# eps696/aphantasia

Hardware: AMD Instinct MI355X
Metric: optimization steps/sec @1280x720 ViT-B/32 samples=200 (higher is better)
Workload: dtype f16 (MFMA operands, fp32 accumulate; fp32 residual stream / LayerNorm / softmax statistics / synth / sampler / loss / Adam)

## Files before the change

### aphantasia_amd/_ffi.py

```python
import ctypes
import os
from ctypes import POINTER, c_char_p, c_float, c_int, c_size_t, c_void_p

import torch

HERE = os.path.dirname(os.path.abspath(__file__))
LIB_PATH = os.path.join(HERE, 'libaphantasia_hip.so')

APH_OUT_NCHW_RAW, APH_OUT_NCHW_NORM, APH_OUT_PATCH_F16, APH_GRAD_PATCH_F16, APH_OUT_PATCH_F16_HILO, APH_OUT_PATCH_F32 = 0, 1, 2, 3, 4, 5
APH_AUG_STRIDE = 16
APH_TF_FAST, APH_TF_CUSTOM, APH_TF_ELASTIC = 0, 1, 2
SIM_TYPES = {'cossim': 0, 'cos': 0, None: 0, 'mix': 1, 'ang': 2, 'dot': 3}


class SampleGeom(ctypes.Structure):
    _fields_ = [(n, c_int) for n in ('H', 'W', 'Hp', 'Wp', 'py0', 'px0', 'S', 'size', 'patch')]


_PROTOTYPES = {
    'aph_version': (c_int, []),
    'aph_last_error': (c_char_p, []),
    'aph_synth_plan_create': (c_int, [c_int, c_int, c_int, POINTER(c_void_p)]),
    'aph_synth_plan_destroy': (c_int, [c_void_p]),
    'aph_synth_fft_fwd': (c_int, [c_void_p, c_void_p, c_void_p, c_void_p, c_float, POINTER(c_float), c_int, c_void_p, c_void_p, c_void_p]),
    'aph_synth_fft_bwd': (c_int, [c_void_p, c_void_p, c_float, c_void_p, c_void_p, c_void_p, c_float, POINTER(c_float), c_int, c_void_p, c_void_p]),
    'aph_irfft2': (c_int, [c_void_p, c_void_p, c_void_p, c_void_p]),
    'aph_rfft2': (c_int, [c_void_p, c_void_p, c_void_p, c_void_p]),
    'aph_synth_spatial_fwd': (c_int, [c_void_p, c_void_p, c_float, c_float, POINTER(c_float), c_int, c_void_p, c_void_p]),
    'aph_synth_spatial_bwd': (c_int, [c_void_p, c_void_p, c_float, c_void_p, c_void_p, c_float, c_float, POINTER(c_float), c_int, c_void_p, c_void_p]),
    'aph_synth_stats': (c_int, [c_void_p, c_void_p, c_void_p]),
    'aph_synth_set_stats': (c_int, [c_void_p, c_void_p, c_void_p]),
    'aph_synth_plan_describe': (c_int, [c_void_p, POINTER(c_int)]),
    'aph_idwt_coarse_levels': (c_int, [POINTER(c_int), POINTER(c_int), c_int, c_int]),
    'aph_rgb_priors_ws_bytes': (c_size_t, []),
    'aph_rgb_sharp': (c_int, [c_void_p, c_int, c_int, c_float, c_void_p, c_void_p, c_void_p, c_void_p]),
    'aph_rgb_priors': (c_int, [c_void_p, c_int, c_int, c_float, c_float, c_float, c_void_p, c_void_p, c_void_p, c_void_p]),
    'aph_cppn_param_count': (c_size_t, [c_int, c_int, c_int]),
    'aph_cppn_ws_bytes': (c_size_t, [c_int, c_int, c_int, c_int, c_int]),
    'aph_cppn_fwd': (c_int, [c_void_p, c_int, c_int, c_int, c_void_p, c_void_p, c_int, c_int, c_void_p, c_void_p, c_void_p]),
    'aph_cppn_bwd': (c_int, [c_void_p, c_int, c_int, c_int, c_void_p, c_void_p, c_int, c_int, c_void_p, c_float, c_void_p, c_void_p, c_void_p, c_void_p]),
    'aph_idwt_level_fwd': (c_int, [c_void_p, c_int, c_int, c_void_p, c_int, c_int, c_int, c_void_p, c_void_p, c_int, c_float, c_void_p, c_void_p]),
    'aph_idwt_fwd': (c_int, [c_void_p, c_void_p, c_void_p, c_void_p, c_void_p, c_int, c_int, c_void_p, c_void_p, c_int, c_void_p, c_void_p]),
    'aph_idwt_bwd': (c_int, [c_void_p, c_void_p, c_void_p, c_void_p, c_int, c_int, c_void_p, c_void_p, c_int, c_void_p, c_void_p, c_void_p, c_void_p]),
    'aph_idwt_level_bwd': (c_int, [c_void_p, c_int, c_int, c_int, c_void_p, c_void_p, c_int, c_float, c_void_p, c_int, c_int, c_void_p, c_void_p]),
    'aph_sample_ws_bytes': (c_size_t, [POINTER(SampleGeom), c_int]),
    'aph_sample_fwd': (c_int, [POINTER(SampleGeom), c_void_p, c_void_p, c_void_p, c_void_p, c_void_p, c_int, c_void_p]),
    'aph_sample_bwd': (c_int, [POINTER(SampleGeom), c_void_p, c_float, c_void_p, c_void_p, c_void_p, c_void_p, c_int, c_void_p]),
    'aph_sample_ws_bytes_tf': (c_size_t, [POINTER(SampleGeom), c_int]),
    'aph_sample_fwd_tf': (c_int, [POINTER(SampleGeom), c_int, c_void_p, c_void_p, c_void_p, c_void_p, c_void_p, c_void_p, c_int, c_void_p]),
    'aph_sample_bwd_tf': (c_int, [POINTER(SampleGeom), c_int, c_void_p, c_float, c_void_p, c_void_p, c_void_p, c_void_p, c_void_p, c_int, c_void_p]),
    'aph_triangle_blur': (c_int, [c_void_p, c_int, c_int, c_int, c_int, c_float, c_float, c_void_p, c_void_p]),
    'aph_resize_bicubic': (c_int, [c_void_p, c_int, c_int, c_int, c_void_p, c_int, c_int, c_void_p]),
    'aph_flip_w': (c_int, [c_void_p, c_void_p, c_int, c_int, c_int, c_void_p, c_void_p]),
    'aph_grid_warp': (c_int, [c_void_p, c_void_p, c_int, c_int, c_int, c_float, c_float, c_float, c_float, c_float, c_void_p, c_void_p, c_void_p]),
    'aph_attn_test': (c_int, [c_void_p, c_void_p, c_void_p, c_void_p, c_void_p, c_void_p, c_int, c_int, c_int, c_int, c_void_p]),
    'aph_attn_f32_test': (c_int, [c_void_p, c_void_p, c_void_p, c_void_p, c_void_p, c_void_p, c_int, c_int, c_int, c_int, c_void_p]),
    'aph_attn_causal_f32_test': (c_int, [c_void_p, c_void_p, c_void_p, c_int, c_int, c_int, c_void_p]),
    'aph_text_create': (c_int, [c_int, c_int, c_int, c_int, c_int, c_int, c_int, POINTER(c_void_p)]),
    'aph_text_destroy': (c_int, [c_void_p]),
    'aph_text_workspace_bytes': (c_size_t, [c_void_p]),
    'aph_text_set_weight': (c_int, [c_void_p, c_char_p, c_void_p, c_size_t]),
    'aph_text_forward': (c_int, [c_void_p, c_void_p, c_int, c_void_p, c_void_p]),
    'aph_lpips_create': (c_int, [POINTER(c_int), c_int, c_int, POINTER(c_void_p)]),
    'aph_lpips_destroy': (c_int, [c_void_p]),
    'aph_lpips_workspace_bytes': (c_size_t, [c_void_p]),
    'aph_lpips_set_weight': (c_int, [c_void_p, c_char_p, c_void_p, c_size_t]),
    'aph_lpips_set_target': (c_int, [c_void_p, c_void_p, c_int, c_int, c_void_p]),
    'aph_lpips_value_grad': (c_int, [c_void_p, c_void_p, c_void_p, c_void_p, c_void_p, c_void_p]),
    'aph_lpips_value_grad_half': (c_int, [c_void_p, c_void_p, c_void_p, c_void_p, c_void_p, c_void_p]),
    'aph_lpips_pack_test': (c_int, [c_void_p, c_int, c_int, c_int, c_void_p, c_size_t]),
    'aph_lpips_conv_test': (c_int, [c_void_p, c_int, c_int, c_int, c_void_p, c_int, c_void_p, c_int, c_void_p, c_void_p, c_void_p, c_int, c_int, c_void_p]),
    'aph_lpips_pool_test': (c_int, [c_void_p, c_int, c_int, c_int, c_void_p, c_void_p, c_void_p, c_void_p]),
    'aph_lpips_head_test': (c_int, [c_void_p, c_void_p, c_void_p, c_int, c_int, c_float, c_void_p, c_void_p, c_void_p, c_void_p, c_void_p]),
    'aph_lpips_resize_test': (c_int, [c_void_p, c_int, c_int, c_void_p, c_int, c_void_p]),
    'aph_frame_affine': (c_int, [c_void_p, c_int, c_int, c_int, POINTER(c_float), c_void_p, c_void_p]),
    'aph_patchify_f16': (c_int, [c_void_p, c_int, c_int, c_int, c_void_p, c_void_p]),
    'aph_patchify_f16_hilo': (c_int, [c_void_p, c_int, c_int, c_int, c_void_p, c_void_p]),
    'aph_patchify_f32': (c_int, [c_void_p, c_int, c_int, c_int, c_void_p, c_void_p]),
    'aph_unpatchify_f32': (c_int, [c_void_p, c_int, c_int, c_int, c_float, c_void_p, c_void_p]),
    'aph_patch_row_elems': (c_int, [c_int]),
    'aph_patchify_f16_win': (c_int, [c_void_p, c_int, c_int, c_int, c_int, c_void_p, c_void_p]),
    'aph_unpatchify_f32_win': (c_int, [c_void_p, c_int, c_int, c_int, c_int, c_float, c_void_p, c_void_p]),
    'aph_vit_create': (c_int, [c_int, c_int, c_int, c_int, c_int, c_int, c_int, POINTER(c_void_p)]),
    'aph_vit_destroy': (c_int, [c_void_p]),
    'aph_vit_workspace_bytes': (c_size_t, [c_void_p]),
    'aph_vit_set_weight': (c_int, [c_void_p, c_char_p, c_void_p, c_size_t]),
    'aph_vit_forward': (c_int, [c_void_p, c_void_p, c_int, c_void_p, c_void_p]),
    'aph_vit_forward_hilo': (c_int, [c_void_p, c_void_p, c_int, c_void_p, c_void_p]),
    'aph_vit_enable_hilo': (c_int, [c_void_p]),
    'aph_vit_enable_f32': (c_int, [c_void_p]),
    'aph_vit_forward_f32': (c_int, [c_void_p, c_void_p, c_int, c_void_p, c_void_p]),
    'aph_vit_backward_f32': (c_int, [c_void_p, c_void_p, c_int, c_void_p, c_float, c_void_p]),
    'aph_vit_backward': (c_int, [c_void_p, c_void_p, c_int, c_void_p, c_float, c_void_p]),
    'aph_vit_backward_h': (c_int, [c_void_p, c_void_p, c_int, c_void_p, c_float, c_void_p]),
    'aph_vit_profile': (c_int, [c_void_p, c_int]),
    'aph_vit_profile_read': (c_int, [c_void_p, c_void_p, c_void_p, c_void_p]),
    'aph_gemm_set_mfma32': (c_int, [c_int]),
    'aph_vit_set_fuse_ln': (c_int, [c_int]),
    'aph_crop_adjoint_set_gather': (c_int, [c_int]),
    'aph_crop_adjoint_set_shape': (c_int, [c_int, c_int, c_int, c_int, c_int]),
    'aph_vit_set_grad_stream_f16': (c_int, [c_int]),
    'aph_gemm_set_ws_min_tiles': (c_int, [c_int]),
    'aph_gemm_set_ws_pgroup': (c_int, [c_int]),
    'aph_gemm_set_rs': (c_int, [c_int]),
    'aph_mfma_rate': (c_int, [c_int, c_int, c_void_p, c_void_p, c_void_p]),
    'aph_gemm_rs_probe': (c_int, [c_void_p, c_void_p, c_int, c_int, c_int, c_void_p, c_int, c_void_p, c_void_p]),
    'aph_gemm_ws_probe': (c_int, [c_void_p, c_void_p, c_int, c_int, c_int, c_void_p, c_void_p, c_void_p, c_int, c_void_p, c_void_p]),
    'aph_gemm_f32_test': (c_int, [c_void_p, c_int, c_int, c_void_p, c_int, c_int, c_int, c_int, c_void_p, c_int, c_void_p, c_void_p, c_int, c_void_p, c_size_t, c_void_p]),
    'aph_gemm_f16': (c_int, [c_void_p, c_void_p, c_int, c_int, c_int, c_void_p, c_void_p]),
    'aph_gemm_f16_ld': (c_int, [c_void_p, c_int, c_void_p, c_int, c_int, c_int, c_int, c_void_p, c_int, c_void_p]),
    'aph_gemm_f16_epi_test': (c_int, [c_void_p, c_int, c_void_p, c_int, c_int, c_int, c_int, c_void_p, c_int, c_void_p, c_void_p, c_void_p, c_float, c_int,
                                      c_int, c_int, c_int, c_void_p, c_size_t, c_int, c_void_p]),
    'aph_ln_test': (c_int, [c_int, c_int, c_int, c_int, c_int, c_int, c_int, c_void_p, c_void_p, c_void_p, c_void_p, c_void_p, c_void_p, c_void_p,
                            c_void_p, c_void_p, c_void_p, c_void_p, c_void_p, c_void_p, c_void_p]),
    'aph_sim_loss': (c_int, [c_void_p, c_int, c_int, c_void_p, c_void_p, POINTER(c_float), c_int, c_int, c_int, c_int, c_int, c_float, c_float, c_void_p, c_void_p, c_void_p, c_void_p]),
    'aph_axpy_f32': (c_int, [c_void_p, c_void_p, c_float, c_size_t, c_void_p]),
    'aph_rgb_to_u8': (c_int, [c_void_p, c_int, c_int, c_float, c_void_p, c_void_p]),
    'aph_linear_head': (c_int, [c_void_p, c_int, c_int, c_void_p, c_float, c_float, c_float, c_float, c_void_p, c_void_p, c_void_p]),
    'aph_comm_unique_id': (c_int, [c_void_p]),
    'aph_comm_init': (c_int, [c_int, c_int, c_void_p, POINTER(c_void_p)]),
    'aph_allreduce_f32': (c_int, [c_void_p, c_void_p, c_size_t, c_void_p]),
    'aph_comm_ranks': (c_int, [c_void_p, POINTER(c_int)]),
    'aph_comm_destroy': (c_int, [c_void_p]),
    'aph_adam_step': (c_int, [c_void_p, c_void_p, c_void_p, c_void_p, c_void_p, c_void_p, c_int, c_size_t, c_void_p]),
    'aph_adam_step_guarded': (c_int, [c_void_p, c_void_p, c_void_p, c_void_p, c_void_p, c_void_p, c_int, c_size_t, c_void_p, c_void_p]),
}

EXPORTS = tuple(_PROTOTYPES)

class Library:

    def __init__(self, path):
        if not os.path.isfile(path):
            raise RuntimeError(
                "aphantasia_amd: HIP library not found at %s -- build it with "
                "`python -c 'import __graft_entry__ as g; g.build()'` (hipcc, gfx950). "
                "There is no CPU fallback." % path)
        self.path = path
        self.cdll = ctypes.CDLL(path)
        for name, (res, args) in _PROTOTYPES.items():
            fn = getattr(self.cdll, name)
            fn.restype = res
            fn.argtypes = args

    def last_error(self):
        return (self.cdll.aph_last_error() or b'').decode(errors='replace')

    def call(self, name, *args):
        rc = getattr(self.cdll, name)(*args)
        if rc < 0:
            raise RuntimeError('%s failed (%d): %s' % (name, rc, self.last_error()))
        return rc


_lib = None


def lib():
    global _lib
    if _lib is None:
        import torch
        if torch.cuda.is_available():
            torch.cuda.init()
            torch.empty(1, device='cuda')
        _lib = Library(LIB_PATH)
    return _lib


def ptr(t):
    return c_void_p(t.data_ptr()) if t is not None else c_void_p(0)


def floats(seq):
    if seq is None:
        return None
    arr = (c_float * len(seq))(*[float(v) for v in seq])
    return arr
```

### aphantasia_amd/csrc/synth.hip

```cpp
#include "synth_fft.h"
#include "synth_rgb.h"
#include "synth_terms.h"
#include "synth_cppn.h"

#include <memory>

using namespace aph;

static const int kElemBlocks = 1024;

struct aph_synth_plan {
  int C, H, W, Wc, TC, col_threads = 1024;
  Fft1D ph, pw;
  int col_blocks, nrow_blocks;
  size_t col_lds, row_lds;
  float norm;
  float2 *twH = nullptr, *twW = nullptr;
  float2* tmp = nullptr;
  float* dn = nullptr;
  double* partials = nullptr;
  float* stats = nullptr;
  float* bstats = nullptr;
  size_t HW() const { return (size_t)H * W; }
  double n() const { return (double)C * H * W; }
  ~aph_synth_plan() {
    for (void* q : {(void*)twH, (void*)twW, (void*)tmp, (void*)dn, (void*)partials, (void*)stats, (void*)bstats}) (void)hipFree(q);
  }
};

static bool factorize(int n, Fft1D* p) {
  p->n = n; p->npass = 0;
  int m = n;
  auto push = [&](int r) { if (p->npass >= 14) return false; p->radix[p->npass++] = r; return true; };
  while (m % 4 == 0) { if (!push(4)) return false; m /= 4; }
  while (m % 2 == 0) { if (!push(2)) return false; m /= 2; }
  for (int r = 3; (long long)r * r <= m || r <= 31; r += 2)
    while (m % r == 0) { if (!push(r)) return false; m /= r; }
  if (m > 1 && !push(m)) return false;
  return true;
}

template <typename T>
static bool dev_alloc(T** p, size_t n) { return hipMalloc((void**)p, sizeof(T) * n) == hipSuccess; }

static float2* make_twiddles(int n) {
  std::vector<float2> h(n);
  for (int t = 0; t < n; ++t) {
    const double ang = 2.0 * M_PI * (double)t / (double)n;
    h[t] = make_float2((float)cos(ang), (float)sin(ang));
  }
  float2* d = nullptr;
  if (!dev_alloc(&d, n)) return nullptr;
  if (hipMemcpy(d, h.data(), sizeof(float2) * n, hipMemcpyHostToDevice) != hipSuccess) { (void)hipFree(d); return nullptr; }
  return d;
}

static void launch_col_synth(const aph_synth_plan* p, const float* spectrum, const float* scale, const float* shift, hipStream_t st) {
  APH_LAUNCH(fft_col_synth_kernel, dim3(p->col_blocks), dim3(p->col_threads), p->col_lds, st, (const float2*)spectrum, scale, shift, p->tmp,
             p->ph, (const float2*)p->twH, p->C, p->H, p->Wc, p->TC);
}
static void launch_row_synth(const aph_synth_plan* p, float* image, hipStream_t st) {
  APH_LAUNCH(fft_row_synth_kernel, dim3(p->nrow_blocks), dim3(256), p->row_lds, st, (const float2*)p->tmp, image, p->partials, p->pw,
             (const float2*)p->twW, p->H, p->W, p->Wc, p->norm);
}
static void launch_row_adjoint(const aph_synth_plan* p, const float* dn, const float* raw, int plain, hipStream_t st) {
  APH_LAUNCH(fft_row_adjoint_kernel, dim3(p->nrow_blocks), dim3(256), p->row_lds, st, dn, raw, plain ? (const float*)nullptr : (const float*)p->bstats,
             p->tmp, p->pw, (const float2*)p->twW, p->H, p->W, p->Wc, p->norm, plain);
}
static void launch_col_adjoint(const aph_synth_plan* p, const float* scale, float* spectrum, hipStream_t st) {
  APH_LAUNCH(fft_col_adjoint_kernel, dim3(p->col_blocks), dim3(p->col_threads), p->col_lds, st, (const float2*)p->tmp, scale, (float2*)spectrum,
             p->ph, (const float2*)p->twH, p->C, p->H, p->Wc, p->TC);
}
static void launch_stats_finalize(const aph_synth_plan* p, int nparts, hipStream_t st) {
  APH_LAUNCH(stats_finalize_kernel, dim3(1), dim3(256), 0, st, (const double*)p->partials, nparts, p->n(), p->stats);
}

static ColorMat to_cm(const float* cc) { ColorMat m; for (int i = 0; i < 9; ++i) m.m[i] = cc ? cc[i] : (i % 4 == 0 ? 1.f : 0.f); return m; }

static void launch_rgb_fwd(const aph_synth_plan* p, const float* raw, float contrast, float fixed_div, const float* colcorr_t9, int decorrelate,
                           float* rgb, hipStream_t st) {
  APH_LAUNCH(rgb_fwd_kernel, dim3(kElemBlocks), dim3(256), 0, st, raw, (const float*)p->stats, contrast, fixed_div, to_cm(colcorr_t9),
             decorrelate, rgb, p->HW());
}
static void launch_rgb_bwd(const aph_synth_plan* p, const float* d_rgb, float gscale, const float* rgb, const float* raw, float contrast,
                           float fixed_div, const float* colcorr_t9, int decorrelate, hipStream_t st) {
  APH_LAUNCH(rgb_bwd_kernel, dim3(kElemBlocks), dim3(256), 0, st, d_rgb, rgb, raw, to_cm(colcorr_t9), decorrelate, gscale, p->dn,
             p->partials, p->HW());
  APH_LAUNCH(bstats_finalize_kernel, dim3(1), dim3(256), 0, st, (const double*)p->partials, kElemBlocks, p->n(), (const float*)p->stats,
             contrast, fixed_div, p->bstats);
}

struct CppnArgs {
  const float *params, *xs, *ys;
  int W;
  size_t HW;
  CppnLayout g;
  hipStream_t st;
};
template <int ACT>
static void launch_cppn_fwd(const CppnNet& net, const CppnArgs& a, float* stash, float* rgb) {
  const size_t lds = sizeof(float) * net.fwd_lds();
  APH_ALLOW_SMEM(cppn_fwd_kernel<ACT>, lds);
  APH_LAUNCH(cppn_fwd_kernel<ACT>, dim3(a.g.ntiles < kCppnFwdBlocks ? a.g.ntiles : kCppnFwdBlocks), dim3(64 * kCppnWaves), lds, a.st, a.params, net,
             a.xs, a.ys, a.W, a.HW, stash, rgb, a.g.ntiles);
}
template <int ACT>
static void launch_cppn_bwd(const CppnNet& net, const CppnArgs& a, const float* d_rgb, float gscale, const float* rgb, const float* stash,
                            float* partials) {
  const size_t lds = sizeof(float) * net.bwd_lds();
  APH_ALLOW_SMEM(cppn_bwd_kernel<ACT>, lds);
  APH_LAUNCH(cppn_bwd_kernel<ACT>, dim3(a.g.bwd_blocks), dim3(64 * kCppnWaves), lds, a.st, a.params, net, a.xs, a.ys, a.W, a.HW, d_rgb, gscale,
             rgb, stash, partials, net.count(), a.g.ntiles);
}

extern "C" {

int aph_synth_plan_create(int C, int H, int W, aph_synth_plan** out) {
  APH_TRY
  if (!out || C < 1 || H < 2 || W < 2) return aph_fail(APH_ERR_ARG, "aph_synth_plan_create: bad shape C=%d H=%d W=%d", C, H, W);
  std::unique_ptr<aph_synth_plan> p(new aph_synth_plan());
  p->C = C; p->H = H; p->W = W; p->Wc = W / 2 + 1;
  if (!factorize(H, &p->ph) || !factorize(W, &p->pw))
    return aph_fail(APH_ERR_UNSUPPORTED, "FFT size %dx%d has more than 14 prime factors", W, H);
  if (W > 8192 || H > 8192) return aph_fail(APH_ERR_UNSUPPORTED, "FFT dimension > 8192 not supported (%dx%d)", W, H);
  int tc = (64 * 1024) / (H * 8);
  p->TC = tc < 1 ? 1 : (tc > 8 ? 8 : tc);
  p->col_blocks = (C * p->Wc + p->TC - 1) / p->TC;
  p->nrow_blocks = C * ((H + 1) / 2);
  p->col_lds = sizeof(float2) * 2 * p->TC * H;
  p->row_lds = sizeof(float2) * 2 * W;
  p->norm = (float)(1.0 / sqrt((double)H * (double)W));
  const int npart = p->nrow_blocks > kElemBlocks ? p->nrow_blocks : kElemBlocks;
  const bool ok = (p->twH = make_twiddles(H)) && (p->twW = make_twiddles(W)) && dev_alloc(&p->tmp, (size_t)C * H * p->Wc) &&
                  dev_alloc(&p->dn, (size_t)C * H * W) && dev_alloc(&p->partials, 2 * (size_t)npart) && dev_alloc(&p->stats, 2) &&
                  dev_alloc(&p->bstats, 4);
  if (!ok) return aph_fail(APH_ERR_HIP, "synth plan allocation failed");
  APH_ALLOW_SMEM(fft_col_synth_kernel, p->col_lds);
  APH_ALLOW_SMEM(fft_col_adjoint_kernel, p->col_lds);
  APH_ALLOW_SMEM(fft_row_synth_kernel, p->row_lds);
  APH_ALLOW_SMEM(fft_row_adjoint_kernel, p->row_lds);
  *out = p.release();
  return APH_OK;
  APH_CATCH
}

int aph_synth_plan_destroy(aph_synth_plan* p) {
  delete p;
  return APH_OK;
}

int aph_synth_plan_describe(const aph_synth_plan* p, int* out31) {
  APH_TRY
  if (!p || !out31) return aph_fail(APH_ERR_ARG, "aph_synth_plan_describe: null argument");
  out31[0] = p->TC;
  const Fft1D* plans[2] = {&p->ph, &p->pw};
  for (int a = 0; a < 2; ++a) {
    int* o = out31 + 1 + 15 * a;
    o[0] = plans[a]->npass;
    for (int i = 0; i < 14; ++i) o[1 + i] = i < plans[a]->npass ? plans[a]->radix[i] : 0;
  }
  return APH_OK;
  APH_CATCH
}

int aph_synth_fft_fwd(aph_synth_plan* p, const float* params, const float* scale, const float* shift, float contrast,
                      const float* colcorr_t9, int decorrelate, float* raw, float* rgb, void* stream_) {
  APH_TRY
  if (!p || !params || !scale || !raw || !rgb) return aph_fail(APH_ERR_ARG, "aph_synth_fft_fwd: null argument");
  hipStream_t st = (hipStream_t)stream_;
  launch_col_synth(p, params, scale, shift, st);
  launch_row_synth(p, raw, st);
  launch_stats_finalize(p, p->nrow_blocks, st);
  launch_rgb_fwd(p, raw, contrast, 0.f, colcorr_t9, decorrelate, rgb, st);
  return aph_check_launch("aph_synth_fft_fwd");
  APH_CATCH
}

int aph_synth_fft_bwd(aph_synth_plan* p, const float* d_rgb, float gscale, const float* rgb, const float* raw,
                      const float* scale, float contrast, const float* colcorr_t9, int decorrelate, float* grad_params,
                      void* stream_) {
  APH_TRY
  if (!p || !d_rgb || !rgb || !raw || !scale || !grad_params) return aph_fail(APH_ERR_ARG, "aph_synth_fft_bwd: null argument");
  hipStream_t st = (hipStream_t)stream_;
  launch_rgb_bwd(p, d_rgb, gscale, rgb, raw, contrast, 0.f, colcorr_t9, decorrelate, st);
  launch_row_adjoint(p, p->dn, raw, 0, st);
  launch_col_adjoint(p, scale, grad_params, st);
  return aph_check_launch("aph_synth_fft_bwd");
  APH_CATCH
}

int aph_irfft2(aph_synth_plan* p, const float* spectrum, float* image, void* stream_) {
  APH_TRY
  if (!p || !spectrum || !image) return aph_fail(APH_ERR_ARG, "aph_irfft2: null argument");
  hipStream_t st = (hipStream_t)stream_;
  launch_col_synth(p, spectrum, nullptr, nullptr, st);
  launch_row_synth(p, image, st);
  return aph_check_launch("aph_irfft2");
  APH_CATCH
}

int aph_rfft2(aph_synth_plan* p, const float* image, float* spectrum, void* stream_) {
  APH_TRY
  if (!p || !image || !spectrum) return aph_fail(APH_ERR_ARG, "aph_rfft2: null argument");
  hipStream_t st = (hipStream_t)stream_;
  launch_row_adjoint(p, image, image, 1, st);
  launch_col_adjoint(p, nullptr, spectrum, st);
  return aph_check_launch("aph_rfft2");
  APH_CATCH
}

int aph_synth_spatial_fwd(aph_synth_plan* p, const float* raw, float contrast, float fixed_div, const float* colcorr_t9,
                          int decorrelate, float* rgb, void* stream_) {
  APH_TRY
  if (!p || !raw || !rgb) return aph_fail(APH_ERR_ARG, "aph_synth_spatial_fwd: null argument");
  hipStream_t st = (hipStream_t)stream_;
  APH_LAUNCH(stats_partial_kernel, dim3(kElemBlocks, 1), dim3(256), 0, st, raw, (size_t)p->C * p->HW(), p->partials);
  launch_stats_finalize(p, kElemBlocks, st);
  launch_rgb_fwd(p, raw, contrast, fixed_div, colcorr_t9, decorrelate, rgb, st);
  return aph_check_launch("aph_synth_spatial_fwd");
  APH_CATCH
}

int aph_synth_spatial_bwd(aph_synth_plan* p, const float* d_rgb, float gscale, const float* rgb, const float* raw,
                          float contrast, float fixed_div, const float* colcorr_t9, int decorrelate, float* d_raw,
                          void* stream_) {
  APH_TRY
  if (!p || !d_rgb || !rgb || !raw || !d_raw) return aph_fail(APH_ERR_ARG, "aph_synth_spatial_bwd: null argument");
  hipStream_t st = (hipStream_t)stream_;
  launch_rgb_bwd(p, d_rgb, gscale, rgb, raw, contrast, fixed_div, colcorr_t9, decorrelate, st);
  APH_LAUNCH(norm_bwd_kernel, dim3(kElemBlocks), dim3(256), 0, st, (const float*)p->dn, raw, (const float*)p->bstats, d_raw, (size_t)p->C * p->HW());
  return aph_check_launch("aph_synth_spatial_bwd");
  APH_CATCH
}

int aph_synth_stats(aph_synth_plan* p, float* out2, void* stream_) {
  APH_TRY
  if (!p || !out2) return aph_fail(APH_ERR_ARG, "aph_synth_stats: null argument");
  if (hipMemcpyAsync(out2, p->stats, 2 * sizeof(float), hipMemcpyDeviceToDevice, (hipStream_t)stream_) != hipSuccess)
    return aph_fail(APH_ERR_HIP, "aph_synth_stats: copy failed");
  return APH_OK;
  APH_CATCH
}

int aph_synth_set_stats(aph_synth_plan* p, const float* in2, void* stream_) {
  APH_TRY
// ... 78 lines not shown
```

### aphantasia_amd/csrc/synth_fft.h

```cpp
#pragma once
#include "synth_rgb.h"

namespace aph {

struct Fft1D {
  int n, npass;
  int radix[14];
};

__device__ __forceinline__ float2 cmul(float2 a, float2 b) {
  return make_float2(a.x * b.x - a.y * b.y, a.x * b.y + a.y * b.x);
}
__device__ __forceinline__ float2 cadd(float2 a, float2 b) { return make_float2(a.x + b.x, a.y + b.y); }
__device__ __forceinline__ float2 csub(float2 a, float2 b) { return make_float2(a.x - b.x, a.y - b.y); }
template <int SIGN>
__device__ __forceinline__ float2 cmuli(float2 a) {
  return SIGN > 0 ? make_float2(-a.y, a.x) : make_float2(a.y, -a.x);
}
template <int SIGN>
__device__ __forceinline__ float2 twiddle(const float2* __restrict__ tw, int t) {
  float2 w = tw[t];
  if (SIGN < 0) w.y = -w.y;
  return w;
}

struct Butterfly {
  const float2* x;
  float2* y;
  int k;
  __device__ __forceinline__ Butterfly(const float2* src, float2* dst, int N, int R, int Ns, int q, int j)
      : x(src + q * N + j), y(dst + q * N + (j / Ns) * Ns * R + j % Ns), k(j % Ns) {}
};

template <int SIGN, int RT>
__device__ __forceinline__ void fft_pass(const float2* src, float2* dst, int N, int R_, int Ns, int nseq,
                                         const float2* __restrict__ tw) {
  const int R = RT ? RT : R_;
  const int nb = N / R, tscale = N / (Ns * R);
  for (int idx = threadIdx.x; idx < nb * nseq; idx += blockDim.x) {
    const int q = idx / nb;
    const Butterfly bf(src, dst, N, R, Ns, q, idx - q * nb);
    float2 v[RT ? RT : 32];
    for (int r = 0; r < R; ++r) {
      v[r] = bf.x[r * nb];
      if (r > 0) v[r] = cmul(v[r], twiddle<SIGN>(tw, bf.k * r * tscale));
    }
    if (RT == 2) {
      bf.y[0] = cadd(v[0], v[1]);
      bf.y[Ns] = csub(v[0], v[1]);
    } else if (RT == 3) {
      const float2 s = cadd(v[1], v[2]);
      const float2 t = make_float2(v[0].x - 0.5f * s.x, v[0].y - 0.5f * s.y);
      float2 u = csub(v[1], v[2]);
      u = cmuli<SIGN>(make_float2(u.x * 0.86602540378443865f, u.y * 0.86602540378443865f));
      bf.y[0] = cadd(v[0], s);
      bf.y[Ns] = cadd(t, u);
      bf.y[2 * Ns] = csub(t, u);
    } else if (RT == 4) {
      const float2 a0 = cadd(v[0], v[2]), a1 = csub(v[0], v[2]);
      const float2 a2 = cadd(v[1], v[3]), a3 = cmuli<SIGN>(csub(v[1], v[3]));
      bf.y[0] = cadd(a0, a2);
      bf.y[Ns] = cadd(a1, a3);
      bf.y[2 * Ns] = csub(a0, a2);
      bf.y[3 * Ns] = csub(a1, a3);
    } else {
      for (int qq = 0; qq < R; ++qq) {
        float2 acc = v[0];
        for (int r = 1; r < R; ++r) acc = cadd(acc, cmul(v[r], twiddle<SIGN>(tw, ((qq * r) % R) * nb)));
        bf.y[qq * Ns] = acc;
      }
    }
  }
}

template <int SIGN>
__device__ void fft_pass_large(const float2* src, float2* dst, int N, int R, int Ns, int nseq, const float2* __restrict__ tw) {
  const int nb = N / R, tscale = N / (Ns * R);
  for (int idx = threadIdx.x; idx < N * nseq; idx += blockDim.x) {
    const int q = idx / N, o = idx - q * N;
    const int qq = o / nb;
    const Butterfly bf(src, dst, N, R, Ns, q, o - qq * nb);
    const float2* x = bf.x;
    double ar = x[0].x, ai = x[0].y;
    const int step = (int)(((long long)bf.k * tscale + (long long)qq * nb) % N);
    int t = 0;
    for (int r = 1; r < R; ++r) {
      t += step; if (t >= N) t -= N;
      const float2 pr = cmul(x[r * nb], twiddle<SIGN>(tw, t));
      ar += pr.x; ai += pr.y;
    }
    bf.y[qq * Ns] = make_float2((float)ar, (float)ai);
  }
}

template <int SIGN>
__device__ float2* fft_lds(float2* a, float2* b, const Fft1D& plan, int nseq, const float2* __restrict__ tw) {
  int Ns = 1;
  const int N = plan.n;
  for (int p = 0; p < plan.npass; ++p) {
    const int R = plan.radix[p];
    switch (R) {
      case 2: fft_pass<SIGN, 2>(a, b, N, R, Ns, nseq, tw); break;
      case 3: fft_pass<SIGN, 3>(a, b, N, R, Ns, nseq, tw); break;
      case 4: fft_pass<SIGN, 4>(a, b, N, R, Ns, nseq, tw); break;
      case 5: fft_pass<SIGN, 5>(a, b, N, R, Ns, nseq, tw); break;
      default:
        if (R <= 31) fft_pass<SIGN, 0>(a, b, N, R, Ns, nseq, tw);
        else fft_pass_large<SIGN>(a, b, N, R, Ns, nseq, tw);
        break;
    }
    __syncthreads();
    float2* t = a; a = b; b = t;
    Ns *= R;
  }
  return a;
}

constexpr int kLoadBatch = 8;

struct ColElem {
  bool in_tile, valid;
  int lds;
  int plane;
  size_t global;
  __device__ __forceinline__ ColElem(int idx, int C, int H, int Wc, int TC) {
    const int t = idx % TC, y = idx / TC, g = blockIdx.x * TC + t;
    in_tile = idx < TC * H;
    valid = in_tile && g < C * Wc;
    const int c = valid ? g / Wc : 0, kx = valid ? g - c * Wc : 0;
    lds = t * H + y;
    plane = (valid ? y : 0) * Wc + kx;
    global = (size_t)c * H * Wc + plane;
  }
};

struct RowPair {
  size_t row0, row1, row1_or_0;
  bool has1;
  __device__ __forceinline__ explicit RowPair(int H) {
    const int pairs = (H + 1) / 2, c = blockIdx.x / pairs, y0 = 2 * (blockIdx.x - c * pairs);
    has1 = y0 + 1 < H;
    row0 = (size_t)c * H + y0;
    row1 = row0 + 1;
    row1_or_0 = has1 ? row1 : row0;
  }
};

__global__ void fft_col_synth_kernel(const float2* __restrict__ params, const float* __restrict__ scale,
                                     const float* __restrict__ shift, float2* __restrict__ tmp, Fft1D plan,
                                     const float2* __restrict__ tw, int C, int H, int Wc, int TC) {
  APH_DYN_SMEM(smem);
  float2* a = reinterpret_cast<float2*>(smem);
  float2* b = a + TC * H;
  for (int base = 0; base < TC * H; base += kLoadBatch * blockDim.x) {
    float2 v[kLoadBatch];
    float sc[kLoadBatch], sf[kLoadBatch];
#pragma unroll
    for (int u = 0; u < kLoadBatch; ++u) {
      const ColElem e(base + u * blockDim.x + threadIdx.x, C, H, Wc, TC);
      v[u] = params[e.global];
      sc[u] = scale ? scale[e.plane] : 1.0f;
      sf[u] = shift ? shift[e.plane] : 0.f;
    }
#pragma unroll
    for (int u = 0; u < kLoadBatch; ++u) {
      const ColElem e(base + u * blockDim.x + threadIdx.x, C, H, Wc, TC);
      if (e.in_tile) {
        float2 w = make_float2(0.f, 0.f);
        if (e.valid) {
          const float s = sc[u];
          w = v[u];
          w.x *= s; w.y *= s;
          if (shift) { const float sh = s * sf[u]; w.x += sh; w.y += sh; }
        }
        a[e.lds] = w;
      }
    }
  }
  __syncthreads();
  const float2* r = fft_lds<+1>(a, b, plan, TC, tw);
  for (int idx = threadIdx.x; idx < TC * H; idx += blockDim.x) {
    const ColElem e(idx, C, H, Wc, TC);
    if (e.valid) tmp[e.global] = r[e.lds];
  }
}

__global__ void fft_col_adjoint_kernel(const float2* __restrict__ tmp, const float* __restrict__ scale,
                                       float2* __restrict__ grad, Fft1D plan, const float2* __restrict__ tw,
                                       int C, int H, int Wc, int TC) {
  APH_DYN_SMEM(smem);
  float2* a = reinterpret_cast<float2*>(smem);
  float2* b = a + TC * H;
  for (int base = 0; base < TC * H; base += kLoadBatch * blockDim.x) {
    float2 v[kLoadBatch];
#pragma unroll
    for (int u = 0; u < kLoadBatch; ++u) v[u] = tmp[ColElem(base + u * blockDim.x + threadIdx.x, C, H, Wc, TC).global];
#pragma unroll
    for (int u = 0; u < kLoadBatch; ++u) {
      const ColElem e(base + u * blockDim.x + threadIdx.x, C, H, Wc, TC);
      if (e.in_tile) a[e.lds] = e.valid ? v[u] : make_float2(0.f, 0.f);
    }
  }
  __syncthreads();
  const float2* r = fft_lds<-1>(a, b, plan, TC, tw);
  for (int idx = threadIdx.x; idx < TC * H; idx += blockDim.x) {
    const ColElem e(idx, C, H, Wc, TC);
    if (e.valid) {
      const float s = scale ? scale[e.plane] : 1.0f;
      const float2 v = r[e.lds];
      grad[e.global] = make_float2(v.x * s, v.y * s);
    }
  }
}

__global__ void fft_row_synth_kernel(const float2* __restrict__ tmp, float* __restrict__ raw,
                                     double* __restrict__ partials, Fft1D plan, const float2* __restrict__ tw,
                                     int H, int W, int Wc, float norm) {
  APH_DYN_SMEM(smem);
  float2* a = reinterpret_cast<float2*>(smem);
  float2* b = a + W;
  __shared__ double red[16];
  const RowPair rp(H);
  const float2* ra = tmp + rp.row0 * Wc;
  const float2* rb = tmp + rp.row1_or_0 * Wc;
  for (int base = 0; base < Wc; base += kLoadBatch * blockDim.x) {
    float2 Av[kLoadBatch], Bw[kLoadBatch];
#pragma unroll
    for (int u = 0; u < kLoadBatch; ++u) {
      const int k = base + u * blockDim.x + threadIdx.x, kc = k < Wc ? k : 0;
      Av[u] = ra[kc];
      Bw[u] = rb[kc];
    }
#pragma unroll
    for (int u = 0; u < kLoadBatch; ++u) {
      const int k = base + u * blockDim.x + threadIdx.x;
      if (k < Wc) {
        const float2 A = Av[u];
        const float2 Bv = rp.has1 ? Bw[u] : make_float2(0.f, 0.f);
        const bool edge = (k == 0) || (2 * k == W);
        if (edge) {
          a[k] = make_float2(A.x, Bv.x);
        } else {
          a[k] = make_float2(A.x - Bv.y, A.y + Bv.x);
          a[W - k] = make_float2(A.x + Bv.y, Bv.x - A.y);
        }
      }
    }
  }
  __syncthreads();
  const float2* r = fft_lds<+1>(a, b, plan, 1, tw);
  SumSq s;
  float* o0 = raw + rp.row0 * W;
  float* o1 = raw + rp.row1 * W;
  for (int x = threadIdx.x; x < W; x += blockDim.x) {
    const float2 z = r[x];
    const float v0 = z.x * norm, v1 = z.y * norm;
    o0[x] = v0;
    s.add(v0);
    if (rp.has1) { o1[x] = v1; s.add(v1); }
  }
  s.store_block_total(red, partials + 2 * blockIdx.x);
}

__global__ void fft_row_adjoint_kernel(const float* __restrict__ dn, const float* __restrict__ raw,
                                       const float* __restrict__ bstats, float2* __restrict__ tmp, Fft1D plan,
                                       const float2* __restrict__ tw, int H, int W, int Wc, float norm, int plain) {
  APH_DYN_SMEM(smem);
  float2* a = reinterpret_cast<float2*>(smem);
  float2* b = a + W;
  const RowPair rp(H);
  const float A = plain ? 1.0f : bstats[0], Bc = plain ? 0.0f : bstats[1], mu = plain ? 0.0f : bstats[2];
  const size_t o0 = rp.row0 * W, o1c = rp.row1_or_0 * W;
  for (int base = 0; base < W; base += kLoadBatch * blockDim.x) {
    float d0[kLoadBatch], r0[kLoadBatch], d1[kLoadBatch], r1[kLoadBatch];
#pragma unroll
    for (int u = 0; u < kLoadBatch; ++u) {
      const int x = base + u * blockDim.x + threadIdx.x, xc = x < W ? x : 0;
      d0[u] = dn[o0 + xc]; r0[u] = raw[o0 + xc];
      d1[u] = dn[o1c + xc]; r1[u] = raw[o1c + xc];
    }
#pragma unroll
    for (int u = 0; u < kLoadBatch; ++u) {
      const int x = base + u * blockDim.x + threadIdx.x;
      if (x < W) {
        const float g0 = A * d0[u] + Bc * (r0[u] - mu);
        const float g1 = rp.has1 ? A * d1[u] + Bc * (r1[u] - mu) : 0.f;
        a[x] = make_float2(g0, g1);
      }
    }
  }
  __syncthreads();
  const float2* r = fft_lds<-1>(a, b, plan, 1, tw);
  float2* t0 = tmp + rp.row0 * Wc;
  float2* t1 = tmp + rp.row1 * Wc;
  for (int k = threadIdx.x; k < Wc; k += blockDim.x) {
    const float2 z = r[k];
    const float2 zc = r[k == 0 ? 0 : W - k];
    const float f = ((!plain && k >= 1 && k <= W - Wc) ? 1.0f : 0.5f) * norm;
    t0[k] = make_float2((z.x + zc.x) * f, (z.y - zc.y) * f);
    if (rp.has1) t1[k] = make_float2((z.y + zc.y) * f, (zc.x - z.x) * f);
  }
}

}
```

Measured before the change: 178.3.

## Add small-radix FFT path with fast division and LDS-staged twiddles

Adds a templated SMALL variant of the synth column and row FFT kernels for sizes whose radices are all at most 5 (e.g. 720 and 1280). It precomputes magic-multiplier divisors to replace integer division in pass indexing and tile mapping. It stages the twiddle tables into LDS with async global-to-LDS loads, and restructures the column tile so each thread owns one column and strides over rows. This targets index arithmetic and global twiddle reads in the image-parameterisation FFTs, at the cost of extra LDS per block (possibly lower occupancy) and fast-division range checks.

```diff
diff --git a/aphantasia_amd/_ffi.py b/aphantasia_amd/_ffi.py
--- a/aphantasia_amd/_ffi.py
+++ b/aphantasia_amd/_ffi.py
@@ -98,6 +98,7 @@
     'aph_gemm_set_mfma32': (c_int, [c_int]),
     'aph_vit_set_fuse_ln': (c_int, [c_int]),
     'aph_crop_adjoint_set_gather': (c_int, [c_int]),
+    'aph_synth_set_generic_passes': (c_int, [c_int]),
     'aph_crop_adjoint_set_shape': (c_int, [c_int, c_int, c_int, c_int, c_int]),
     'aph_vit_set_grad_stream_f16': (c_int, [c_int]),
     'aph_gemm_set_ws_min_tiles': (c_int, [c_int]),
diff --git a/aphantasia_amd/csrc/synth.hip b/aphantasia_amd/csrc/synth.hip
--- a/aphantasia_amd/csrc/synth.hip
+++ b/aphantasia_amd/csrc/synth.hip
@@ -3,6 +3,8 @@
 #include "synth_terms.h"
 #include "synth_cppn.h"
 
+#include <algorithm>
+#include <initializer_list>
 #include <memory>
 
 using namespace aph;
@@ -14,6 +16,8 @@
   Fft1D ph, pw;
   int col_blocks, nrow_blocks;
   size_t col_lds, row_lds;
+  bool col_small = false, row_small = false;
+  FastDiv by_tc, by_wc, by_pairs;
   float norm;
   float2 *twH = nullptr, *twW = nullptr;
   float2* tmp = nullptr;
@@ -37,16 +41,41 @@
   for (int r = 3; (long long)r * r <= m || r <= 31; r += 2)
     while (m % r == 0) { if (!push(r)) return false; m /= r; }
   if (m > 1 && !push(m)) return false;
+  p->small = 1;
+  for (int i = 0, ns = 1; i < p->npass; ns *= p->radix[i++]) {
+    p->by_nb[i] = fast_div(n / p->radix[i]);
+    p->by_ns[i] = fast_div(ns);
+    if (p->radix[i] > 5) p->small = 0;
+  }
+  return true;
+}
+
+static bool fast_div_holds(FastDiv d, unsigned long long n_end) { return d.d == 1 || n_end * d.d <= (1ull << 32); }
+
+static const size_t kLdsBytes = 160 * 1024;
+
+static int& generic_passes() {
+  static int v = 0;
+  return v;
+}
+
+static bool small_plan(const Fft1D& f, size_t lds, unsigned long long idx_end, std::initializer_list<FastDiv> dividers) {
+  if (!f.small || lds + sizeof(float2) * tw_padded(f.n) > kLdsBytes) return false;
+  for (int i = 0; i < f.npass; ++i)
+    if (!fast_div_holds(f.by_nb[i], idx_end) || !fast_div_holds(f.by_ns[i], idx_end)) return false;
+  for (FastDiv d : dividers)
+    if (!fast_div_holds(d, idx_end)) return false;
   return true;
 }
 
 template <typename T>
 static bool dev_alloc(T** p, size_t n) { return hipMalloc((void**)p, sizeof(T) * n) == hipSuccess; }
 
-static float2* make_twiddles(int n) {
-  std::vector<float2> h(n);
-  for (int t = 0; t < n; ++t) {
-    const double ang = 2.0 * M_PI * (double)t / (double)n;
+static float2* make_twiddles(int n_) {
+  const int n = tw_padded(n_);
+  std::vector<float2> h(n, make_float2(0.f, 0.f));
+  for (int t = 0; t < n_; ++t) {
+    const double ang = 2.0 * M_PI * (double)t / (double)n_;
     h[t] = make_float2((float)cos(ang), (float)sin(ang));
   }
   float2* d = nullptr;
@@ -55,21 +84,29 @@
   return d;
 }
 
+#define APH_LAUNCH_FFT(kern, small, ...)                            \
+  do {                                                              \
+    if ((small) && !generic_passes()) { APH_LAUNCH(kern<true>, __VA_ARGS__); } \
+    else { APH_LAUNCH(kern<false>, __VA_ARGS__); }                  \
+  } while (0)
+static ColTile col_tile(const aph_synth_plan* p) { return ColTile{p->C, p->H, p->Wc, p->TC, p->col_threads / p->TC, p->by_tc, p->by_wc}; }
+
 static void launch_col_synth(const aph_synth_plan* p, const float* spectrum, const float* scale, const float* shift, hipStream_t st) {
-  APH_LAUNCH(fft_col_synth_kernel, dim3(p->col_blocks), dim3(p->col_threads), p->col_lds, st, (const float2*)spectrum, scale, shift, p->tmp,
-             p->ph, (const float2*)p->twH, p->C, p->H, p->Wc, p->TC);
+  APH_LAUNCH_FFT(fft_col_synth_kernel, p->col_small, dim3(p->col_blocks), dim3(p->col_threads), p->col_lds, st, (const float2*)spectrum, scale,
+                 shift, p->tmp, p->ph, (const float2*)p->twH, col_tile(p));
 }
 static void launch_row_synth(const aph_synth_plan* p, float* image, hipStream_t st) {
-  APH_LAUNCH(fft_row_synth_kernel, dim3(p->nrow_blocks), dim3(256), p->row_lds, st, (const float2*)p->tmp, image, p->partials, p->pw,
-             (const float2*)p->twW, p->H, p->W, p->Wc, p->norm);
+  APH_LAUNCH_FFT(fft_row_synth_kernel, p->row_small, dim3(p->nrow_blocks), dim3(256), p->row_lds, st, (const float2*)p->tmp, image, p->partials,
+                 p->pw, (const float2*)p->twW, p->H, p->W, p->Wc, p->norm, p->by_pairs);
 }
 static void launch_row_adjoint(const aph_synth_plan* p, const float* dn, const float* raw, int plain, hipStream_t st) {
-  APH_LAUNCH(fft_row_adjoint_kernel, dim3(p->nrow_blocks), dim3(256), p->row_lds, st, dn, raw, plain ? (const float*)nullptr : (const float*)p->bstats,
-             p->tmp, p->pw, (const float2*)p->twW, p->H, p->W, p->Wc, p->norm, plain);
+  APH_LAUNCH_FFT(fft_row_adjoint_kernel, p->row_small, dim3(p->nrow_blocks), dim3(256), p->row_lds, st, dn, raw,
+                 plain ? (const float*)nullptr : (const float*)p->bstats, p->tmp, p->pw, (const float2*)p->twW, p->H, p->W, p->Wc, p->norm, plain,
+                 p->by_pairs);
 }
 static void launch_col_adjoint(const aph_synth_plan* p, const float* scale, float* spectrum, hipStream_t st) {
-  APH_LAUNCH(fft_col_adjoint_kernel, dim3(p->col_blocks), dim3(p->col_threads), p->col_lds, st, (const float2*)p->tmp, scale, (float2*)spectrum,
-             p->ph, (const float2*)p->twH, p->C, p->H, p->Wc, p->TC);
+  APH_LAUNCH_FFT(fft_col_adjoint_kernel, p->col_small, dim3(p->col_blocks), dim3(p->col_threads), p->col_lds, st, (const float2*)p->tmp, scale,
+                 (float2*)spectrum, p->ph, (const float2*)p->twH, col_tile(p));
 }
 static void launch_stats_finalize(const aph_synth_plan* p, int nparts, hipStream_t st) {
   APH_LAUNCH(stats_finalize_kernel, dim3(1), dim3(256), 0, st, (const double*)p->partials, nparts, p->n(), p->stats);
@@ -129,16 +166,23 @@
   p->nrow_blocks = C * ((H + 1) / 2);
   p->col_lds = sizeof(float2) * 2 * p->TC * H;
   p->row_lds = sizeof(float2) * 2 * W;
+  p->by_tc = fast_div(p->TC); p->by_wc = fast_div(p->Wc); p->by_pairs = fast_div((H + 1) / 2);
+  const unsigned long long col_end = std::max<unsigned long long>({(unsigned long long)p->col_threads, (unsigned long long)p->TC * H,
+                                                                   (unsigned long long)C * p->Wc + p->TC});
+  p->col_small = small_plan(p->ph, p->col_lds, col_end, {p->by_tc, p->by_wc});
+  p->row_small = small_plan(p->pw, p->row_lds, std::max<unsigned long long>(W, p->nrow_blocks), {p->by_pairs});
+  if (p->col_small) p->col_lds += sizeof(float2) * tw_padded(H);
+  if (p->row_small) p->row_lds += sizeof(float2) * tw_padded(W);
   p->norm = (float)(1.0 / sqrt((double)H * (double)W));
   const int npart = p->nrow_blocks > kElemBlocks ? p->nrow_blocks : kElemBlocks;
   const bool ok = (p->twH = make_twiddles(H)) && (p->twW = make_twiddles(W)) && dev_alloc(&p->tmp, (size_t)C * H * p->Wc) &&
                   dev_alloc(&p->dn, (size_t)C * H * W) && dev_alloc(&p->partials, 2 * (size_t)npart) && dev_alloc(&p->stats, 2) &&
                   dev_alloc(&p->bstats, 4);
   if (!ok) return aph_fail(APH_ERR_HIP, "synth plan allocation failed");
-  APH_ALLOW_SMEM(fft_col_synth_kernel, p->col_lds);
-  APH_ALLOW_SMEM(fft_col_adjoint_kernel, p->col_lds);
-  APH_ALLOW_SMEM(fft_row_synth_kernel, p->row_lds);
-  APH_ALLOW_SMEM(fft_row_adjoint_kernel, p->row_lds);
+  APH_ALLOW_SMEM(fft_col_synth_kernel<true>, p->col_lds);   APH_ALLOW_SMEM(fft_col_synth_kernel<false>, p->col_lds);
+  APH_ALLOW_SMEM(fft_col_adjoint_kernel<true>, p->col_lds); APH_ALLOW_SMEM(fft_col_adjoint_kernel<false>, p->col_lds);
+  APH_ALLOW_SMEM(fft_row_synth_kernel<true>, p->row_lds);   APH_ALLOW_SMEM(fft_row_synth_kernel<false>, p->row_lds);
+  APH_ALLOW_SMEM(fft_row_adjoint_kernel<true>, p->row_lds); APH_ALLOW_SMEM(fft_row_adjoint_kernel<false>, p->row_lds);
   *out = p.release();
   return APH_OK;
   APH_CATCH
@@ -161,6 +205,12 @@
   }
   return APH_OK;
   APH_CATCH
+}
+
+int aph_synth_set_generic_passes(int on) {
+  const int prev = generic_passes();
+  generic_passes() = on ? 1 : 0;
+  return prev;
 }
 
 int aph_synth_fft_fwd(aph_synth_plan* p, const float* params, const float* scale, const float* shift, float contrast,
diff --git a/aphantasia_amd/csrc/synth_fft.h b/aphantasia_amd/csrc/synth_fft.h
--- a/aphantasia_amd/csrc/synth_fft.h
+++ b/aphantasia_amd/csrc/synth_fft.h
@@ -2,10 +2,18 @@
 #include "synth_rgb.h"
 
 namespace aph {
+
+struct FastDiv {
+  uint32_t d, m;
+  __host__ __device__ __forceinline__ int quot(int n) const { return d == 1 ? n : (int)(((uint64_t)(uint32_t)n * m) >> 32); }
+};
+inline FastDiv fast_div(int d) { return FastDiv{(uint32_t)d, d > 1 ? (uint32_t)((1ull << 32) / (uint32_t)d) + 1u : 0u}; }
 
 struct Fft1D {
   int n, npass;
   int radix[14];
+  FastDiv by_nb[14], by_ns[14];
+  int small;
 };
 
 __device__ __forceinline__ float2 cmul(float2 a, float2 b) {
@@ -93,21 +101,81 @@
   }
 }
 
-template <int SIGN>
-__device__ float2* fft_lds(float2* a, float2* b, const Fft1D& plan, int nseq, const float2* __restrict__ tw) {
+template <int SIGN, int R>
+__device__ __forceinline__ void fft_pass_small(const float2* src, float2* dst, int N, int Ns, int nseq, const float2* tw, FastDiv by_nb,
+                                               FastDiv by_ns) {
+  const int nb = (int)by_nb.d, tscale = by_ns.quot(nb);
+  float2 root[R];
+  if (R == 5) {
+#pragma unroll
+    for (int m = 0; m < R; ++m) root[m] = twiddle<SIGN>(tw, m * nb);
+  }
+  for (int idx = threadIdx.x; idx < nb * nseq; idx += blockDim.x) {
+    const int q = nseq == 1 ? 0 : by_nb.quot(idx), j = idx - q * nb;
+    const int blk = by_ns.quot(j), k = j - blk * Ns;
+    const float2* x = src + q * N + j;
+    float2* y = dst + q * N + blk * Ns * R + k;
+    float2 v[R];
+#pragma unroll
+    for (int r = 0; r < R; ++r) {
+      v[r] = x[r * nb];
+      if (r > 0) v[r] = cmul(v[r], twiddle<SIGN>(tw, k * r * tscale));
+    }
+    if (R == 2) {
+      y[0] = cadd(v[0], v[1]);
+      y[Ns] = csub(v[0], v[1]);
+    } else if (R == 3) {
+      const float2 s = cadd(v[1], v[2]);
+      const float2 t = make_float2(v[0].x - 0.5f * s.x, v[0].y - 0.5f * s.y);
+      float2 u = csub(v[1], v[2]);
+      u = cmuli<SIGN>(make_float2(u.x * 0.86602540378443865f, u.y * 0.86602540378443865f));
+      y[0] = cadd(v[0], s);
+      y[Ns] = cadd(t, u);
+      y[2 * Ns] = csub(t, u);
+    } else if (R == 4) {
+      const float2 a0 = cadd(v[0], v[2]), a1 = csub(v[0], v[2]);
+      const float2 a2 = cadd(v[1], v[3]), a3 = cmuli<SIGN>(csub(v[1], v[3]));
+      y[0] = cadd(a0, a2);
+      y[Ns] = cadd(a1, a3);
+      y[2 * Ns] = csub(a0, a2);
+      y[3 * Ns] = csub(a1, a3);
+    } else {
+#pragma unroll
+      for (int qq = 0; qq < R; ++qq) {
+        float2 acc = v[0];
+#pragma unroll
+        for (int r = 1; r < R; ++r) acc = cadd(acc, cmul(v[r], root[(qq * r) % R]));
+        y[qq * Ns] = acc;
+      }
+    }
+  }
+}
+
+template <int SIGN, bool SMALL>
+__device__ float2* fft_lds(float2* a, float2* b, const Fft1D& plan, int nseq, const float2* tw) {
   int Ns = 1;
   const int N = plan.n;
   for (int p = 0; p < plan.npass; ++p) {
     const int R = plan.radix[p];
-    switch (R) {
-      case 2: fft_pass<SIGN, 2>(a, b, N, R, Ns, nseq, tw); break;
-      case 3: fft_pass<SIGN, 3>(a, b, N, R, Ns, nseq, tw); break;
-      case 4: fft_pass<SIGN, 4>(a, b, N, R, Ns, nseq, tw); break;
-      case 5: fft_pass<SIGN, 5>(a, b, N, R, Ns, nseq, tw); break;
-      default:
-        if (R <= 31) fft_pass<SIGN, 0>(a, b, N, R, Ns, nseq, tw);
-        else fft_pass_large<SIGN>(a, b, N, R, Ns, nseq, tw);
-        break;
+    if (SMALL) {
+      const FastDiv by_nb = plan.by_nb[p], by_ns = plan.by_ns[p];
+      switch (R) {
+        case 2: fft_pass_small<SIGN, 2>(a, b, N, Ns, nseq, tw, by_nb, by_ns); break;
+        case 3: fft_pass_small<SIGN, 3>(a, b, N, Ns, nseq, tw, by_nb, by_ns); break;
+        case 4: fft_pass_small<SIGN, 4>(a, b, N, Ns, nseq, tw, by_nb, by_ns); break;
+        default: fft_pass_small<SIGN, 5>(a, b, N, Ns, nseq, tw, by_nb, by_ns); break;
+      }
+    } else {
+      switch (R) {
+        case 2: fft_pass<SIGN, 2>(a, b, N, R, Ns, nseq, tw); break;
+        case 3: fft_pass<SIGN, 3>(a, b, N, R, Ns, nseq, tw); break;
+        case 4: fft_pass<SIGN, 4>(a, b, N, R, Ns, nseq, tw); break;
+        case 5: fft_pass<SIGN, 5>(a, b, N, R, Ns, nseq, tw); break;
+        default:
+          if (R <= 31) fft_pass<SIGN, 0>(a, b, N, R, Ns, nseq, tw);
+          else fft_pass_large<SIGN>(a, b, N, R, Ns, nseq, tw);
+          break;
+      }
     }
     __syncthreads();
     float2* t = a; a = b; b = t;
@@ -118,27 +186,58 @@
 
 constexpr int kLoadBatch = 8;
 
-struct ColElem {
-  bool in_tile, valid;
-  int lds;
-  int plane;
-  size_t global;
-  __device__ __forceinline__ ColElem(int idx, int C, int H, int Wc, int TC) {
-    const int t = idx % TC, y = idx / TC, g = blockIdx.x * TC + t;
-    in_tile = idx < TC * H;
-    valid = in_tile && g < C * Wc;
-    const int c = valid ? g / Wc : 0, kx = valid ? g - c * Wc : 0;
-    lds = t * H + y;
-    plane = (valid ? y : 0) * Wc + kx;
-    global = (size_t)c * H * Wc + plane;
-  }
-};
-
+template <bool SMALL>
+__device__ __forceinline__ int quot(int n, FastDiv d) { return SMALL ? d.quot(n) : n / (int)d.d; }
+
+constexpr int kTwChunk = 128;
+__host__ __device__ __forceinline__ int tw_padded(int n) { return (n + kTwChunk - 1) / kTwChunk * kTwChunk; }
+template <bool SMALL>
+__device__ __forceinline__ const float2* stage_twiddles(const float2* __restrict__ tw, float2* lds, int n) {
+  if (!SMALL) return tw;
+  const int wave = wave_uniform(threadIdx.x >> 6), nw = blockDim.x >> 6, lane = threadIdx.x & 63;
+  for (int c = wave * kTwChunk; c < n; c += nw * kTwChunk) glds16(tw + c + 2 * lane, lds + c);
+  return lds;
+}
+__device__ __forceinline__ void wait_twiddles() {
+#ifndef APH_EMU
+  asm volatile("s_waitcnt vmcnt(0)" ::: "memory");
+#endif
+}
+
+struct ColTile {
+  int C, H, Wc, TC, rows;
+  FastDiv by_tc, by_wc;
+};
+
+template <bool SMALL>
+struct ColThread {
+  bool active, valid;
+  int y0, rows, H, Wc;
+  int lds0;
+  int kx;
+  size_t global0;
+  __device__ __forceinline__ explicit ColThread(const ColTile& g) : rows(g.rows), H(g.H), Wc(g.Wc) {
+    y0 = quot<SMALL>(threadIdx.x, g.by_tc);
+    const int t = threadIdx.x - y0 * g.TC, col = blockIdx.x * g.TC + t;
+    active = y0 < rows;
+    valid = active && col < g.C * g.Wc;
+    const int c = valid ? quot<SMALL>(col, g.by_wc) : 0;
+    kx = valid ? col - c * g.Wc : 0;
+    lds0 = t * g.H;
+    global0 = (size_t)c * g.H * g.Wc + kx;
+  }
+  __device__ __forceinline__ bool has(int y) const { return active && y < H; }
+  __device__ __forceinline__ int lds(int y) const { return lds0 + y; }
+  __device__ __forceinline__ int plane(int y) const { return y * Wc + kx; }
+  __device__ __forceinline__ size_t global(int y) const { return global0 + (size_t)(y * Wc); }
+};
+
+template <bool SMALL>
 struct RowPair {
   size_t row0, row1, row1_or_0;
   bool has1;
-  __device__ __forceinline__ explicit RowPair(int H) {
-    const int pairs = (H + 1) / 2, c = blockIdx.x / pairs, y0 = 2 * (blockIdx.x - c * pairs);
+  __device__ __forceinline__ RowPair(int H, FastDiv by_pairs) {
+    const int c = quot<SMALL>(blockIdx.x, by_pairs), y0 = 2 * (blockIdx.x - c * (int)by_pairs.d);
     has1 = y0 + 1 < H;
     row0 = (size_t)c * H + y0;
     row1 = row0 + 1;
@@ -146,90 +245,102 @@
   }
 };
 
+template <bool SMALL>
 __global__ void fft_col_synth_kernel(const float2* __restrict__ params, const float* __restrict__ scale,
                                      const float* __restrict__ shift, float2* __restrict__ tmp, Fft1D plan,
-                                     const float2* __restrict__ tw, int C, int H, int Wc, int TC) {
+                                     const float2* __restrict__ tw, ColTile g) {
   APH_DYN_SMEM(smem);
   float2* a = reinterpret_cast<float2*>(smem);
-  float2* b = a + TC * H;
-  for (int base = 0; base < TC * H; base += kLoadBatch * blockDim.x) {
+  float2* b = a + g.TC * g.H;
+  const float2* twp = stage_twiddles<SMALL>(tw, b + g.TC * g.H, g.H);
+  const ColThread<SMALL> ct(g);
+  for (int base = ct.y0; base < g.H; base += kLoadBatch * ct.rows) {
     float2 v[kLoadBatch];
     float sc[kLoadBatch], sf[kLoadBatch];
 #pragma unroll
     for (int u = 0; u < kLoadBatch; ++u) {
-      const ColElem e(base + u * blockDim.x + threadIdx.x, C, H, Wc, TC);
-      v[u] = params[e.global];
-      sc[u] = scale ? scale[e.plane] : 1.0f;
-      sf[u] = shift ? shift[e.plane] : 0.f;
-    }
-#pragma unroll
-    for (int u = 0; u < kLoadBatch; ++u) {
-      const ColElem e(base + u * blockDim.x + threadIdx.x, C, H, Wc, TC);
-      if (e.in_tile) {
+      const int y = base + u * ct.rows;
+      if (ct.valid && y < g.H) {
+        v[u] = params[ct.global(y)];
+        sc[u] = scale ? scale[ct.plane(y)] : 1.0f;
+        sf[u] = shift ? shift[ct.plane(y)] : 0.f;
+      }
+    }
+#pragma unroll
+    for (int u = 0; u < kLoadBatch; ++u) {
+      const int y = base + u * ct.rows;
+      if (ct.has(y)) {
         float2 w = make_float2(0.f, 0.f);
-        if (e.valid) {
+        if (ct.valid) {
           const float s = sc[u];
           w = v[u];
           w.x *= s; w.y *= s;
           if (shift) { const float sh = s * sf[u]; w.x += sh; w.y += sh; }
         }
-        a[e.lds] = w;
-      }
-    }
-  }
+        a[ct.lds(y)] = w;
+      }
+    }
+  }
+  wait_twiddles();
   __syncthreads();
-  const float2* r = fft_lds<+1>(a, b, plan, TC, tw);
-  for (int idx = threadIdx.x; idx < TC * H; idx += blockDim.x) {
-    const ColElem e(idx, C, H, Wc, TC);
-    if (e.valid) tmp[e.global] = r[e.lds];
-  }
-}
-
+  const float2* r = fft_lds<+1, SMALL>(a, b, plan, g.TC, twp);
+  if (ct.valid)
+    for (int y = ct.y0; y < g.H; y += ct.rows) tmp[ct.global(y)] = r[ct.lds(y)];
+}
+
+template <bool SMALL>
 __global__ void fft_col_adjoint_kernel(const float2* __restrict__ tmp, const float* __restrict__ scale,
-                                       float2* __restrict__ grad, Fft1D plan, const float2* __restrict__ tw,
-                                       int C, int H, int Wc, int TC) {
+                                       float2* __restrict__ grad, Fft1D plan, const float2* __restrict__ tw, ColTile g) {
   APH_DYN_SMEM(smem);
   float2* a = reinterpret_cast<float2*>(smem);
-  float2* b = a + TC * H;
-  for (int base = 0; base < TC * H; base += kLoadBatch * blockDim.x) {
+  float2* b = a + g.TC * g.H;
+  const float2* twp = stage_twiddles<SMALL>(tw, b + g.TC * g.H, g.H);
+  const ColThread<SMALL> ct(g);
+  for (int base = ct.y0; base < g.H; base += kLoadBatch * ct.rows) {
     float2 v[kLoadBatch];
 #pragma unroll
-    for (int u = 0; u < kLoadBatch; ++u) v[u] = tmp[ColElem(base + u * blockDim.x + threadIdx.x, C, H, Wc, TC).global];
-#pragma unroll
-    for (int u = 0; u < kLoadBatch; ++u) {
-      const ColElem e(base + u * blockDim.x + threadIdx.x, C, H, Wc, TC);
-      if (e.in_tile) a[e.lds] = e.valid ? v[u] : make_float2(0.f, 0.f);
-    }
-  }
+    for (int u = 0; u < kLoadBatch; ++u) {
+      const int y = base + u * ct.rows;
+      if (ct.valid && y < g.H) v[u] = tmp[ct.global(y)];
+    }
+#pragma unroll
+    for (int u = 0; u < kLoadBatch; ++u) {
+      const int y = base + u * ct.rows;
+      if (ct.has(y)) a[ct.lds(y)] = ct.valid ? v[u] : make_float2(0.f, 0.f);
+    }
+  }
+  wait_twiddles();
   __syncthreads();
-  const float2* r = fft_lds<-1>(a, b, plan, TC, tw);
-  for (int idx = threadIdx.x; idx < TC * H; idx += blockDim.x) {
-    const ColElem e(idx, C, H, Wc, TC);
-    if (e.valid) {
-      const float s = scale ? scale[e.plane] : 1.0f;
-      const float2 v = r[e.lds];
-      grad[e.global] = make_float2(v.x * s, v.y * s);
-    }
-  }
-}
-
+  const float2* r = fft_lds<-1, SMALL>(a, b, plan, g.TC, twp);
+  if (ct.valid)
+    for (int y = ct.y0; y < g.H; y += ct.rows) {
+      const float s = scale ? scale[ct.plane(y)] : 1.0f;
+      const float2 v = r[ct.lds(y)];
+      grad[ct.global(y)] = make_float2(v.x * s, v.y * s);
+    }
+}
+
+template <bool SMALL>
 __global__ void fft_row_synth_kernel(const float2* __restrict__ tmp, float* __restrict__ raw,
                                      double* __restrict__ partials, Fft1D plan, const float2* __restrict__ tw,
-                                     int H, int W, int Wc, float norm) {
+                                     int H, int W, int Wc, float norm, FastDiv by_pairs) {
   APH_DYN_SMEM(smem);
   float2* a = reinterpret_cast<float2*>(smem);
   float2* b = a + W;
   __shared__ double red[16];
-  const RowPair rp(H);
+  const RowPair<SMALL> rp(H, by_pairs);
   const float2* ra = tmp + rp.row0 * Wc;
   const float2* rb = tmp + rp.row1_or_0 * Wc;
+  const float2* twp = stage_twiddles<SMALL>(tw, b + W, W);
   for (int base = 0; base < Wc; base += kLoadBatch * blockDim.x) {
     float2 Av[kLoadBatch], Bw[kLoadBatch];
 #pragma unroll
     for (int u = 0; u < kLoadBatch; ++u) {
-      const int k = base + u * blockDim.x + threadIdx.x, kc = k < Wc ? k : 0;
-      Av[u] = ra[kc];
-      Bw[u] = rb[kc];
+      const int k = base + u * blockDim.x + threadIdx.x;
+      if (k < Wc) {
+        Av[u] = ra[k];
+        Bw[u] = rb[k];
+      }
     }
 #pragma unroll
     for (int u = 0; u < kLoadBatch; ++u) {
@@ -247,8 +358,9 @@
       }
     }
   }
+  wait_twiddles();
   __syncthreads();
-  const float2* r = fft_lds<+1>(a, b, plan, 1, tw);
+  const float2* r = fft_lds<+1, SMALL>(a, b, plan, 1, twp);
   SumSq s;
   float* o0 = raw + rp.row0 * W;
   float* o1 = raw + rp.row1 * W;
@@ -262,22 +374,26 @@
   s.store_block_total(red, partials + 2 * blockIdx.x);
 }
 
+template <bool SMALL>
 __global__ void fft_row_adjoint_kernel(const float* __restrict__ dn, const float* __restrict__ raw,
                                        const float* __restrict__ bstats, float2* __restrict__ tmp, Fft1D plan,
-                                       const float2* __restrict__ tw, int H, int W, int Wc, float norm, int plain) {
+                                       const float2* __restrict__ tw, int H, int W, int Wc, float norm, int plain, FastDiv by_pairs) {
   APH_DYN_SMEM(smem);
   float2* a = reinterpret_cast<float2*>(smem);
   float2* b = a + W;
-  const RowPair rp(H);
+  const RowPair<SMALL> rp(H, by_pairs);
   const float A = plain ? 1.0f : bstats[0], Bc = plain ? 0.0f : bstats[1], mu = plain ? 0.0f : bstats[2];
   const size_t o0 = rp.row0 * W, o1c = rp.row1_or_0 * W;
+  const float2* twp = stage_twiddles<SMALL>(tw, b + W, W);
   for (int base = 0; base < W; base += kLoadBatch * blockDim.x) {
     float d0[kLoadBatch], r0[kLoadBatch], d1[kLoadBatch], r1[kLoadBatch];
 #pragma unroll
     for (int u = 0; u < kLoadBatch; ++u) {
-      const int x = base + u * blockDim.x + threadIdx.x, xc = x < W ? x : 0;
-      d0[u] = dn[o0 + xc]; r0[u] = raw[o0 + xc];
-      d1[u] = dn[o1c + xc]; r1[u] = raw[o1c + xc];
+      const int x = base + u * blockDim.x + threadIdx.x;
+      if (x < W) {
+        d0[u] = dn[o0 + x]; r0[u] = raw[o0 + x];
+        d1[u] = dn[o1c + x]; r1[u] = raw[o1c + x];
+      }
     }
 #pragma unroll
     for (int u = 0; u < kLoadBatch; ++u) {
@@ -289,8 +405,9 @@
       }
     }
   }
+  wait_twiddles();
   __syncthreads();
-  const float2* r = fft_lds<-1>(a, b, plan, 1, tw);
+  const float2* r = fft_lds<-1, SMALL>(a, b, plan, 1, twp);
   float2* t0 = tmp + rp.row0 * Wc;
   float2* t1 = tmp + rp.row1 * Wc;
   for (int k = threadIdx.x; k < Wc; k += blockDim.x) {
```

Result: no change. 177.7 (-0.3%).
